# Opendigitalradio/ODR-AudioEnc

Measured on AMD Instinct MI355X. Metric: real-time stereo DAB MP2 streams sustained (frames/s) @128 kbps/48 kHz, higher is better.
Workload: dtype f64; 1 GPU; 4096 streams/GPU x 48 kHz stereo (mode 's') x 128 kbps, psy 1, full encode (BASELINE configs[1]), 32 frames/stream/step; streams_per_gpu=4096, parallelism=streams sharded over 1 GPU(s), no data-path collective

## Files before the change

### odr-audioenc_amd/csrc/mp2_alloc.h

```cpp
#ifndef MP2_WAVE_PARTS
#error "include mp2_wave.h"
#endif
TL_FN int tl_allocate(const TlBlockShared *TL_RESTRICT B, int adb, int nch, int sblimit, int jsbound, PARG(int, a_ln), PARG(int, a_nbal),
                      PARG(int, a_sfs), PARG(int, a_sfs_o), PARG(double, a_smr), PARG(int, ba))
{
    PV(uint64_t, ukey); PV(uint64_t, ukey2); PV(int, nbits); PV(int, cost); PV(int, cost2);
    PV(int, jpair);
    TL_LANES_BEGIN
    const int c = lane & 1, sb = lane >> 1;
    const bool live = c < nch && sb < sblimit;
    const int maxa = (1 << L(a_nbal)) - 1;
    L(ukey) = live ? tl_mnr_key(B->snr_line[L(a_ln)][0] - L(a_smr)) : ~0ull;
    L(ukey2) = (live && 1 < maxa) ? tl_mnr_key(B->snr_line[L(a_ln)][1] - L(a_smr)) : ~0ull;
    L(ba) = 0;
    L(nbits) = (sb < sblimit && c < (sb < jsbound ? nch : 1)) ? L(a_nbal) : 0;
    L(cost) = live ? B->bits12_line[L(a_ln)][1] + 2 + L(a_sfs) + ((nch == 2 && sb >= jsbound) ? 2 + L(a_sfs_o) : 0) : 0;
    L(cost2) = live ? B->bits12_line[L(a_ln)][2] - B->bits12_line[L(a_ln)][1] : 0;
    L(jpair) = (live && nch == 2 && sb >= jsbound) ? 1 : 0;
    TL_LANES_END
    const int bbal = TL_WAVE_SUM_I32(nbits);
    const int ad = adb - (bbal + 16 + 32);
    int spent = 0;
    const bool any_pair = nch == 2 && jsbound < sblimit;
    for (; TL_ENC_LEVEL < 4;) {
        PV(uint64_t, keff); PV(uint64_t, k2eff);
        TL_LANES_BEGIN L(keff) = L(ukey); L(k2eff) = L(ukey2); TL_LANES_END
        if (any_pair) {
            PV(uint64_t, ok1); PV(uint64_t, ok2);
            TL_SWAP1_U64(ok1, ukey); TL_SWAP1_U64(ok2, ukey2);
            TL_LANES_BEGIN
            if (L(jpair)) { if (L(ok1) < L(keff)) L(keff) = L(ok1); if (L(ok2) < L(k2eff)) L(k2eff) = L(ok2); }
            TL_LANES_END
        }
        const uint64_t M = TL_WAVE_MIN_U64(k2eff);
        PV(bool, inb); PV(int, bcost);
        TL_LANES_BEGIN
        L(inb) = L(keff) < M;
        L(bcost) = (L(inb) && !(L(jpair) && (lane & 1))) ? L(cost) : 0;
        TL_LANES_END
        const uint64_t bm = TL_BALLOT(inb);
        if (bm == 0ull) break;
        const int csum = TL_WAVE_SUM_I32(bcost);
        bool last_round = false;
        if (csum > ad - spent) {
            PV(int, pre); PV(int, kh); PV(int, kl); PV(uint64_t, kb);
            TL_LANES_BEGIN L(pre) = 0; L(kh) = (int)(uint32_t)(L(keff) >> 32); L(kl) = (int)(uint32_t)L(keff); L(kb) = L(keff) + 1; TL_LANES_END
            uint64_t pm = bm;
            while (pm) {
                const int j = __builtin_ctzll(pm);
                pm &= pm - 1;
                const int cj = TL_READLANE_I32(bcost, j);
                if (cj == 0) continue;
                const uint64_t kj = ((uint64_t)(uint32_t)TL_READLANE_I32(kh, j) << 32) | (uint32_t)TL_READLANE_I32(kl, j);
                TL_LANES_BEGIN
                if (kj < L(kb)) L(pre) += cj;
                TL_LANES_END
            }
            TL_LANES_BEGIN
            L(inb) = L(inb) && L(pre) <= ad - spent;
            L(bcost) = L(inb) ? L(bcost) : 0;
            TL_LANES_END
            if (TL_BALLOT(inb) == 0ull) break;
            spent += TL_WAVE_SUM_I32(bcost);
            last_round = true;
        } else spent += csum;
        TL_LANES_BEGIN
        if (L(inb)) {
            const int nba = L(ba) + 1;
            L(ba) = nba;
            L(ukey) = L(ukey2);
            L(cost) = L(cost2);
            L(ukey2) = (nba + 1 >= (1 << L(a_nbal)) - 1) ? ~0ull : tl_mnr_key(B->snr_line[L(a_ln)][(nba + 1) & 15] - L(a_smr));
            L(cost2) = B->bits12_line[L(a_ln)][(nba + 2) & 15] - B->bits12_line[L(a_ln)][(nba + 1) & 15];
        }
        TL_LANES_END
        if (last_round) break;
    }
    for (; TL_ENC_LEVEL < 4;) {
        PV(uint64_t, key);
        TL_LANES_BEGIN
        L(key) = L(cost) <= ad - spent ? L(ukey) : ~0ull;
        TL_LANES_END
        const int wl = TL_WAVE_ARGMIN_U64(key);
        if (wl < 0) break;
        const int min_sb = wl >> 1;
        spent += TL_READLANE_I32(cost, wl);
        const bool joint_pair = (min_sb >= jsbound && nch == 2);
        TL_LANES_BEGIN
        if (lane == wl || (joint_pair && (lane ^ 1) == wl)) {
            const int nba = L(ba) + 1;
            L(ba) = nba;
            L(ukey) = L(ukey2);
            L(cost) = L(cost2);
            L(ukey2) = (nba + 1 >= (1 << L(a_nbal)) - 1) ? ~0ull : tl_mnr_key(B->snr_line[L(a_ln)][(nba + 1) & 15] - L(a_smr));
            L(cost2) = B->bits12_line[L(a_ln)][(nba + 2) & 15] - B->bits12_line[L(a_ln)][(nba + 1) & 15];
        }
        TL_LANES_END
    }
    return ad - spent;
}

TL_FN void tl_allocate_pair(const TlBlockShared *TL_RESTRICT B, int adb0, int adb1, int sblimit, PARG(int, a_ln), PARG(int, a_nbal),
                            PARG(int, a_sfs), PARG(double, a_smr), PARG(int, ba))
{
    PV(uint64_t, ukey); PV(uint64_t, ukey2); PV(int, nbits); PV(int, cost); PV(int, cost2); PV(int, room); PV(int, ph); PV(int, bbal);
    TL_LANES_BEGIN
    const bool live = (lane >> 1) < sblimit;
    const int maxa = (1 << L(a_nbal)) - 1;
    L(ukey) = live ? tl_mnr_key(B->snr_line[L(a_ln)][0] - L(a_smr)) : ~0ull;
    L(ukey2) = (live && 1 < maxa) ? tl_mnr_key(B->snr_line[L(a_ln)][1] - L(a_smr)) : ~0ull;
    L(ba) = 0;
    L(nbits) = live ? L(a_nbal) : 0;
    L(cost) = live ? B->bits12_line[L(a_ln)][1] + 2 + L(a_sfs) : 0;
    L(cost2) = live ? B->bits12_line[L(a_ln)][2] - B->bits12_line[L(a_ln)][1] : 0;
    TL_LANES_END
    TL_PAR_SUM_I32(bbal, nbits);
    TL_LANES_BEGIN
    L(room) = ((lane & 1) ? adb1 : adb0) - (L(bbal) + 16 + 32);
    L(ph) = 0;
    TL_LANES_END
    for (; TL_ENC_LEVEL < 4;) {
        PV(uint64_t, k2); PV(uint64_t, M); PV(bool, inb); PV(int, bcost); PV(int, csum); PV(bool, part);
        TL_LANES_BEGIN L(k2) = L(ph) == 0 ? L(ukey2) : ~0ull; TL_LANES_END
        TL_PAR_MIN_U64(M, k2);
        TL_LANES_BEGIN
        L(inb) = L(ph) == 0 && L(ukey) < L(M);
        L(bcost) = L(inb) ? L(cost) | 0x10000 : 0;
        TL_LANES_END
        if (TL_BALLOT(inb) == 0ull) break;
        TL_PAR_SUM_I32(csum, bcost);
        TL_LANES_BEGIN L(part) = L(ph) == 0 && (L(csum) & 0xffff) > L(room); TL_LANES_END
        if (TL_BALLOT(part) != 0ull) {
            PV(int, pre); PV(int, kh); PV(int, kl); PV(bool, pin);
            TL_LANES_BEGIN
            L(pre) = 0; L(kh) = (int)(uint32_t)(L(ukey) >> 32); L(kl) = (int)(uint32_t)L(ukey); L(pin) = L(inb) && L(part);
            TL_LANES_END
            PV(uint64_t, kb);
            for (int u = 0; u < 2; u++) {
                TL_LANES_BEGIN L(kb) = (lane & 1) == u ? L(ukey) + 1 : 0ull; TL_LANES_END
                uint64_t pm = TL_BALLOT(pin) & (0x5555555555555555ull << u);
                while (pm) {
                    const int j = __builtin_ctzll(pm);
                    pm &= pm - 1;
                    const int cj = TL_READLANE_I32(bcost, j) & 0xffff;
                    const uint64_t kj = ((uint64_t)(uint32_t)TL_READLANE_I32(kh, j) << 32) | (uint32_t)TL_READLANE_I32(kl, j);
                    TL_LANES_BEGIN
                    if (kj < L(kb)) L(pre) += cj;
                    TL_LANES_END
                }
            }
            TL_LANES_BEGIN
            if (L(part)) { L(inb) = L(inb) && L(pre) <= L(room); L(bcost) = L(inb) ? L(bcost) : 0; }
            TL_LANES_END
            TL_PAR_SUM_I32(csum, bcost);
        }
        TL_LANES_BEGIN
        if (L(ph) == 0) {
            L(room) -= L(csum) & 0xffff;
            if ((L(csum) >> 16) == 0 || L(part)) L(ph) = 1;
// ... 35 lines not shown
```

### odr-audioenc_amd/csrc/mp2_pack.h

```cpp
#ifndef MP2_WAVE_PARTS
#error "include mp2_wave.h"
#endif
struct TlFrameOut { uint8_t *bytes; uint32_t *words; uint8_t *scfcrc; };
template <int PSY, int NCH = 0>
TL_FN void tl_encode_frame(TlMainLds &w, const TlTables *TL_RESTRICT T, const TlBlockShared *TL_RESTRICT B,
                           const TlConfig *TL_RESTRICT C, const TlPsyOut *TL_RESTRICT PO,
                           const TlPcmView &pv, int xpad_len, const TlFrameOut &fo,
                           const double *TL_RESTRICT enw_s, const TlPackTables *TL_RESTRICT K, int padding, TlTaps *taps, long long *sp)
{
    constexpr int FB = TlMainLds::kFbBatch;
    const int nch = NCH ? NCH : C->nch, sblimit = C->sblimit;
    PA(double, smp, 36);
    PA(int, scf, 3);

    TL_STAMP(sp, 0);
    TL_PRIO2(TL_PS_FB);
    tl_filterbank(w, B, enw_s, nch, smp);

    TL_STAMP(sp, 1);
    TL_PRIO2(1);
#if !defined(TL_EMULATE) && TL_ENC_LEVEL >= 5
    for (int b = 0; b < 36; b++) TL_KEEP(smp[b]);
    scf[0] = scf[1] = scf[2] = 0;
#endif
// ... 81 lines not shown
            w.smr[c][sb] = top - m;
        }
        TL_LANES_END
    }

    TL_STAMP(sp, 3);
    TL_LANES_BEGIN
    const int c = lane & 1, sb = lane >> 1;
    if (TL_ENC_LEVEL < 5 && c < nch && sb < sblimit) {
        int s0 = L(scf)[0], s1 = L(scf)[1], s2 = L(scf)[2];
        int d0 = s0 - s1, d1 = s1 - s2;
        int c0 = d0 <= -3 ? 0 : d0 < 0 ? 1 : d0 == 0 ? 2 : d0 < 3 ? 3 : 4;
        int c1 = d1 <= -3 ? 0 : d1 < 0 ? 1 : d1 == 0 ? 2 : d1 < 3 ? 3 : 4;
        const unsigned p = B->sfpat[c0 * 5 + c1];
        const int m02 = s0 > s2 ? s2 : s0;
        const unsigned q0 = p & 3u, q1 = (p >> 2) & 3u, q2 = (p >> 4) & 3u;
        const int n0 = q0 == 0 ? s0 : q0 == 1 ? s1 : q0 == 2 ? s2 : m02;
        const int n1 = q1 == 0 ? s0 : q1 == 1 ? s1 : q1 == 2 ? s2 : m02;
        const int n2 = q2 == 0 ? s0 : q2 == 1 ? s1 : q2 == 2 ? s2 : m02;
        const int sel = (int)(p >> 6);
        s0 = n0; s1 = n1; s2 = n2;
        L(scf)[0] = s0; L(scf)[1] = s1; L(scf)[2] = s2;
        w.scf[c][0][sb] = (uint8_t)s0; w.scf[c][1][sb] = (uint8_t)s1; w.scf[c][2][sb] = (uint8_t)s2;
        w.scfsi[c][sb] = (uint8_t)sel;
    } else w.scfsi[c][sb] = 0;
    w.balloc[c][sb] = 0;
    TL_LANES_END

    const int lg_frame = C->frame_bytes + padding;
    int adb = lg_frame * 8 - (C->dab_ext * 8 + (xpad_len ? xpad_len : 2) * 8);
    int mode = C->mode0, mode_ext = C->mode_ext0, jsbound = C->jsbound0;
    PV(int, a_sfs); PV(int, a_sfs_o); PV(double, a_smr); PV(double, a_smr_o);
    TL_LANES_BEGIN
    const int c = lane & 1, sb = lane >> 1;
    const bool live = c < nch && sb < sblimit;
    L(a_sfs) = live ? 6 * tl_sfs_count(w.scfsi[c][sb]) : 0;
    L(a_sfs_o) = (live && nch == 2) ? 6 * tl_sfs_count(w.scfsi[1 - c][sb]) : 0;
    L(a_smr) = live ? w.smr[c][sb] : 0.0;
    L(a_smr_o) = (live && nch == 2) ? w.smr[1 - c][sb] : 0.0;
    TL_LANES_END
    if (TL_ENC_LEVEL < 4 && C->mode0 == 1) {
        PV(int, nz_own); PV(int, nz_jnt);
        TL_LANES_BEGIN
        int bo = 0, bj = 0;
        if (lane < 2 * sblimit) {
            const int ln = L(a_ln), maxAlloc = (1 << L(a_nbal)) - 1;
            double sv[15];
#pragma unroll
            for (int q = 0; q < 15; q++) sv[q] = B->snr_line[ln][q];
            int n1 = 0, n2 = 0;
#pragma unroll
            for (int q = 0; q < 15; q++) {
                const bool inr = q < maxAlloc - 1;
                n1 += (inr && !((sv[q] - L(a_smr)) >= 0.0)) ? 1 : 0;
                n2 += (inr && !((sv[q] - L(a_smr_o)) >= 0.0)) ? 1 : 0;
            }
            n2 = n2 > n1 ? n2 : n1;
            bo = n1 > 0 ? B->bits12_line[ln][n1] + 2 + L(a_sfs) : 0;
            bj = n2 > 0 ? B->bits12_line[ln][n2] + 4 + L(a_sfs) + L(a_sfs_o) : 0;
        }
        L(nz_own) = bo; L(nz_jnt) = bj;
        TL_LANES_END
        mode = 0; mode_ext = 0; jsbound = sblimit;
        int tries = 0, try_ext = 4;
        for (;;) {
            PV(int, need);
            TL_LANES_BEGIN
            const int c = lane & 1, sb = lane >> 1;
            int bitsn = 0;
            if (sb < sblimit && c < (sb < jsbound ? nch : 1))
                bitsn = ((nch == 2 && sb >= jsbound) ? L(nz_jnt) : L(nz_own)) + L(a_nbal);
            L(need) = bitsn;
            TL_LANES_END
            int rq = 32 + 16 + TL_WAVE_SUM_I32(need);
            if (tries == 0) {
                if (rq > adb) { mode = 1; } else break;
            } else if (!(rq > adb && try_ext > 0)) { mode_ext = try_ext; break; }
            --try_ext; jsbound = 4 * (try_ext + 1); tries++;
        }
    }
    int adb_left;
    {
        PV(int, ba);
        adb_left = tl_allocate(B, adb, nch, sblimit, jsbound, a_ln, a_nbal, a_sfs, a_sfs_o, a_smr, ba);
        TL_LANES_BEGIN
        const int c = lane & 1, sb = lane >> 1;
        w.balloc[c][sb] = (uint8_t)((c < nch && sb < sblimit) ? L(ba) : 0);
        TL_LANES_END
    }

    TL_STAMP(sp, 4);
    uint32_t *frame = w.u.frame[0];
    TL_LANES_BEGIN
    for (int i = lane; i < ((lg_frame + 3) >> 2) + 2; i += 64) frame[i] = 0;
    TL_LANES_END
    PV(int, f_ba); PV(int, f_sel); PV(int, f_scf); PV(int, f_smp);
    PV(int, o_ba); PV(int, o_sel); PV(int, o_scf); PV(int, o_smp);
    TL_LANES_BEGIN
    const int c = lane & 1, sb = lane >> 1;
    const bool live = c < nch && sb < sblimit;
    const int ba = live ? w.balloc[c][sb] : 0;
    const bool own = sb < sblimit && c < (sb < jsbound ? nch : 1);
    L(f_ba) = own ? L(a_nbal) : 0;
    L(f_sel) = (live && ba) ? 2 : 0;
    L(f_scf) = (live && ba) ? 6 * tl_sfs_count(w.scfsi[c][sb]) : 0;
    L(f_smp) = (own && ba) ? B->bits12_line[L(a_ln)][ba] / 12 : 0;
    TL_LANES_END
    TL_WAVE_EXSCAN_I32(o_ba, f_ba); TL_WAVE_EXSCAN_I32(o_sel, f_sel);
    TL_WAVE_EXSCAN_I32(o_scf, f_scf); TL_WAVE_EXSCAN_I32(o_smp, f_smp);
    const int n_ba = TL_WAVE_SUM_I32(f_ba), n_sel = TL_WAVE_SUM_I32(f_sel);
    const int n_scf = TL_WAVE_SUM_I32(f_scf), n_smp = TL_WAVE_SUM_I32(f_smp);
    const int p_ba = 48, p_sel = p_ba + n_ba, p_scf = p_sel + n_sel, p_smp = p_scf + n_scf;

    if (TL_ENC_LEVEL < 3) {
    TL_LANES_BEGIN
    const int c = lane & 1, sb = lane >> 1;
    if (lane == 0) {
        uint32_t h = (0xfffu << 20) | ((uint32_t)C->version << 19) | (2u << 17) | (0u << 16)
                   | ((uint32_t)C->br_idx << 12) | ((uint32_t)C->fs_idx << 10) | ((uint32_t)padding << 9) | (0u << 8)
                   | ((uint32_t)mode << 6) | ((uint32_t)mode_ext << 4);
        TL_ATOMIC_OR(&frame[0], h);
    }
    const bool live = c < nch && sb < sblimit;
    const int ba = live ? w.balloc[c][sb] : 0;
    if (L(f_ba)) tl_put_bits48(frame, p_ba + L(o_ba), (uint64_t)ba, L(f_ba));
    if (L(f_sel)) {
        const unsigned si = w.scfsi[c][sb];
        tl_put_bits48(frame, p_sel + L(o_sel), si, 2);
        const unsigned s0 = (unsigned)L(scf)[0], s1 = (unsigned)L(scf)[1], s2 = (unsigned)L(scf)[2];
        const unsigned f3 = (s0 << 12) | (s1 << 6) | s2, f2 = (s0 << 6) | s2;
        tl_put_bits48(frame, p_scf + L(o_scf), si == 0 ? f3 : si == 2 ? s0 : f2, L(f_scf));
    }
    TL_LANES_END
    }

    TL_PRIO2(TL_PS_Q);
    if (TL_ENC_LEVEL < 2) {
        const bool any_joint = (nch == 2) && jsbound < sblimit;
        PV(int, q_ba); PV(int, q_nb); PV(int, q_grp); PV(int, q_s2n); PV(int, q_steps);
        PV(double, q_a); PV(double, q_b); PV(double, q_s2nf); PA(double, q_sf, 3); PA(double, q_rsf, 3);
        TL_LANES_BEGIN
        const int c = lane & 1, sb = lane >> 1;
        const bool own = sb < sblimit && c < (sb < jsbound ? nch : 1);
        const int ba = own ? w.balloc[c][sb] : 0;
        const unsigned qi = ba ? B->qinfo_line[L(a_ln)][ba] : 0u;
        const int q = (int)(qi & 31u);
        const bool joint = any_joint && sb >= jsbound;
        L(q_ba) = ba; L(q_nb) = (int)((qi >> 5) & 31u); L(q_grp) = ((qi >> 10) & 1u) ? 3 : 1; L(q_s2n) = K->steps2n[q];
        L(q_steps) = ((qi >> 10) & 1u) ? 1 << L(q_nb) : K->steps[q];
        L(q_a) = K->qa[q]; L(q_b) = K->qb[q]; L(q_s2nf) = K->steps2n_f[q];
        for (int gr = 0; gr < 3; gr++) {
            L(q_sf)[gr] = B->scalefactor[joint ? w.jscale[gr][sb] : L(scf)[gr]];
            L(q_rsf)[gr] = 1.0 / L(q_sf)[gr];
        }
        TL_LANES_END
        uint64_t q_mask = 0;
        int q_n = 64;
        if (TL_Q_REDEAL && !any_joint && !taps) {
            PV(bool, q_live);
            TL_LANES_BEGIN L(q_live) = L(q_ba) != 0; TL_LANES_END
            q_mask = TL_BALLOT(q_live);
            q_n = (int)__builtin_popcountll(q_mask);
        }
        const bool redeal = q_n <= TL_Q_REDEAL_MAX;
        TL_DBG_REDEAL(redeal, q_ba);
        if (redeal) {
            TlQCell *const qc = TL_QRD_CELLS(w);
// ... 521 lines not shown
```

### odr-audioenc_amd/csrc/mp2_probe_stage.h

```cpp
#pragma once
#include "mp2_host.h"
#include "mp2_wave.h"

enum {
    TLS_ADD_DB = 0,
    TLS_MASK,
    TLS_MNR_KEY,
    TLS_SF_INDEX,
    TLS_DIV_BY,
    TLS_LANE_FORMS,
    TLS_SPANS = TLS_LANE_FORMS,
    TLS_MIN_ROWS,
    TLS_BITS,
    TLS_ALLOC,
    TLS_NFORMS
};
#define TLS_LIST 192
#define TLS_ROWS 136
#define TLS_FIELDS 6
#define TLS_FRAME_WORDS (TL_MAX_FRAME_WORDS + 2)
#define TLS_CRC16_POLY 0x8005u
#define TLS_CRC16_TOP 0x8000u
#define TLS_CRC8_POLY 0x1du
#define TLS_CRC8_TOP 0x80u
// ... 205 lines not shown
TL_FN void tl_probe_stage_case(int form, TlStageLds &w, long k, const void *in0, const void *in1, const void *in2, void *out0, void *out1)
{
    const int32_t *ic = (const int32_t *)in2;
    switch (form) {
    case TLS_SPANS: {
        const double *list = (const double *)in0 + TLS_LIST * k, *bnd = (const double *)in1 + 128 * k;
        const int ntone = TL_UNI_I(ic[2 * k]), nnoise = TL_UNI_I(ic[2 * k + 1]), nm = ntone + nnoise;
        TL_LANES_BEGIN
        for (int q = lane; q < TL_MASKER_MAX; q += 64) TL_MK_X(w)[q] = 0.0;
        for (int q = lane; q < TLS_LIST; q += 64) TL_MK_BARK(w)[q] = list[q];
        TL_LANES_END
        TL_LANES_BEGIN
        for (int t = lane; t < TL_MASKER_MAX; t += 64) {
            if (t < nm) tl_masker_consts(TL_MK4(w), TL_MK_X(w), TL_MK_BARK(w), t, t < ntone);
            else TL_MK4(w)[t].bark = TL_MK_BARK(w)[t];
        }
        TL_LANES_END
        const bool sorted = tl_maskers_sorted(TL_MK_BARK(w), ntone, nnoise);
        const bool srt = ntone < 128 && nnoise < 64 && sorted;
        TL_LANES_BEGIN
        const double blo = bnd[2 * lane], bhi = bnd[2 * lane + 1];
        int32_t *o = (int32_t *)out0 + 512 * k + 8 * lane;
        int a0, a1, b0, b1;
        tl_mask_spans(TL_MK4(w), nm, ntone, blo, bhi, a0, a1, b0, b1);
        o[0] = a0; o[1] = a1; o[2] = b0; o[3] = b1;
        a0 = a1 = b0 = b1 = -2;
        if (srt) tl_mask_spans_sorted<64, 32>(TL_MK_BARK(w), ntone, nnoise, blo, bhi, a0, a1, b0, b1);
        o[4] = a0; o[5] = a1; o[6] = b0; o[7] = b1;
        if (lane == 0) { ((int32_t *)out1)[2 * k] = sorted ? 1 : 0; ((int32_t *)out1)[2 * k + 1] = srt ? 1 : 0; }
        TL_LANES_END
    } break;
    case TLS_MIN_ROWS: {
        const double *col = (const double *)in0 + TLS_ROWS * k, *m0 = (const double *)in1 + 64 * k;
        TL_LANES_BEGIN
        for (int q = lane; q < TLS_ROWS; q += 64) TL_LTG(w)[q] = col[q];
        TL_LANES_END
        TL_LANES_BEGIN
        const int32_t *r = ic + 192 * k + 3 * lane;
        ((double *)out0)[64 * k + lane] = tl_min_rows(TL_LTG(w), r[0], r[1], m0[lane], r[2] != 0);
        TL_LANES_END
    } break;
    case TLS_BITS: {
        const uint64_t *val = (const uint64_t *)in0 + 64 * TLS_FIELDS * k;
        const int32_t *len = (const int32_t *)in1 + 64 * TLS_FIELDS * k;
        const int start = TL_UNI_I(ic[2 * k]), wide = TL_UNI_I(ic[2 * k + 1]);
        uint32_t *frame = w.frame;
        PV(int, tot); PV(int, off);
        TL_LANES_BEGIN
        for (int q = lane; q < TLS_FRAME_WORDS; q += 64) frame[q] = 0;
        int t = 0;
        for (int f = 0; f < TLS_FIELDS; f++) t += len[TLS_FIELDS * lane + f];
        L(tot) = t;
        TL_LANES_END
        TL_WAVE_EXSCAN_I32(off, tot);
        TL_LANES_BEGIN
        int pos = start + L(off);
        unsigned c16 = 0xffffu, c8 = 0;
        for (int f = 0; f < TLS_FIELDS; f++) {
            const uint64_t v = val[TLS_FIELDS * lane + f];
            const int nb = len[TLS_FIELDS * lane + f];
            if (wide) { if (nb) tl_put_bits48(frame, pos, v, nb); }
            else tl_put_bits(frame, pos, (uint32_t)v, nb);
            const int hi = nb > 32 ? nb - 32 : 0;
            c16 = tl_crc_upd(c16, (unsigned)(v >> 32), hi, TLS_CRC16_POLY, TLS_CRC16_TOP); c16 = tl_crc_upd(c16, (unsigned)v, nb - hi, TLS_CRC16_POLY, TLS_CRC16_TOP);
            c8 = tl_crc_upd(c8, (unsigned)(v >> 32), hi, TLS_CRC8_POLY, TLS_CRC8_TOP); c8 = tl_crc_upd(c8, (unsigned)v, nb - hi, TLS_CRC8_POLY, TLS_CRC8_TOP);
            pos += nb;
        }
        ((uint32_t *)out1)[128 * k + 2 * lane] = c16 & 0xffffu; ((uint32_t *)out1)[128 * k + 2 * lane + 1] = c8 & 0xffu;
        TL_LANES_END
        TL_LANES_BEGIN
        uint32_t *o = (uint32_t *)out0 + 3 * TLS_FRAME_WORDS * k;
        for (int q = lane; q < TLS_FRAME_WORDS; q += 64) {
            const uint32_t word = frame[q];
            uint32_t u = 0;
            for (int bit = 0; bit < 32; bit++) u = (u << 1) | tl_get_bit(frame, 32 * q + bit);
            o[q] = word; o[TLS_FRAME_WORDS + q] = u; o[2 * TLS_FRAME_WORDS + q] = tl_bswap(word);
        }
        TL_LANES_END
    } break;
    default: break;
    }
}

TL_FN void tl_probe_alloc_case(const TlBlockShared *TL_RESTRICT B, const TlsAllocTab *TL_RESTRICT A, long k, const void *in0, const void *in1, const void *in2, void *out0, void *out1)
{
    const int32_t *ic = (const int32_t *)in2;
    const double *smr = (const double *)in0 + 64 * k;
    const int32_t *sel = (const int32_t *)in1 + 64 * k, *p = ic + 8 * k;
    const int tab = TL_UNI_I(p[0]), nch = TL_UNI_I(p[1]), jsbound = TL_UNI_I(p[2]), call = TL_UNI_I(p[3]), adb0 = TL_UNI_I(p[4]), adb1 = TL_UNI_I(p[5]);
    const int sblimit = TL_UNI_I(A->sblimit[tab]);
    PV(int, a_ln); PV(int, a_nbal); PV(int, a_sfs); PV(int, a_sfs_o); PV(double, a_smr); PV(int, ba);
    int left = 0;
    if (call == 0) {
        TL_LANES_BEGIN
        const int c = lane & 1, sb = lane >> 1;
        const bool live = c < nch && sb < sblimit;
        L(a_ln) = live ? A->line[tab][sb] : 0;
        L(a_nbal) = live ? A->nbal[tab][sb] : 0;
        L(a_sfs) = live ? 6 * tl_sfs_count((unsigned)sel[lane]) : 0;
        L(a_sfs_o) = (live && nch == 2) ? 6 * tl_sfs_count((unsigned)sel[lane ^ 1]) : 0;
        L(a_smr) = live ? smr[lane] : 0.0;
        TL_LANES_END
        left = tl_allocate(B, adb0, nch, sblimit, jsbound, a_ln, a_nbal, a_sfs, a_sfs_o, a_smr, ba);
    } else {
        TL_LANES_BEGIN
        const int sb = lane >> 1;
        const bool live = sb < sblimit;
        L(a_ln) = live ? A->line[tab][sb] : 0;
        L(a_nbal) = live ? A->nbal[tab][sb] : 0;
        L(a_sfs) = live ? 6 * tl_sfs_count((unsigned)sel[lane]) : 0;
        L(a_smr) = live ? smr[lane] : 0.0;
        TL_LANES_END
        tl_allocate_pair(B, adb0, adb1, sblimit, a_ln, a_nbal, a_sfs, a_smr, ba);
    }
    TL_LANES_BEGIN
    ((int32_t *)out0)[64 * k + lane] = L(ba);
    if (lane == 0) ((int32_t *)out1)[k] = left;
    TL_LANES_END
}
```

### odr-audioenc_amd/csrc/mp2_wave.h

```cpp
#pragma once
#include "mp2_types.h"
#include "tl_libm.h"
#include <math.h>
#include <stddef.h>

#ifdef TL_EMULATE
#define TL_FN static inline
#define TL_LANES_BEGIN for (int lane = 0; lane < 64; ++lane) {
#define TL_LANES_END }
#define TL_SYNC() ((void)0)
#define PV(T, name) T name[64]
#define PA(T, name, n) T name[64][n]
#define L(name) name[lane]
#define PARG(T, name) T (&name)[64]
#define PARGA(T, name, n) T (&name)[64][n]
#define TL_OTHER(name, idx, src) name[src] idx
#define TL_ATOMIC_OR(p, v) (*(p) |= (v))
TL_FN uint64_t tlh_ballot(const bool (&p)[64]) { uint64_t m = 0; for (int i = 0; i < 64; i++) if (p[i]) m |= 1ull << i; return m; }
TL_FN uint64_t tlh_min_u64(const uint64_t (&v)[64]) { uint64_t m = v[0]; for (int i = 1; i < 64; i++) if (v[i] < m) m = v[i]; return m; }
TL_FN int tlh_sum_i32(const int (&v)[64]) { int s = 0; for (int i = 0; i < 64; i++) s += v[i]; return s; }
TL_FN uint32_t tlh_xor_u32(const uint32_t (&v)[64]) { uint32_t s = 0; for (int i = 0; i < 64; i++) s ^= v[i]; return s; }
TL_FN void tlh_exscan_i32(int (&d)[64], const int (&v)[64]) { int s = 0; for (int i = 0; i < 64; i++) { d[i] = s; s += v[i]; } }
TL_FN int tlh_argmin_u64(const uint64_t (&v)[64])
{
    const uint64_t m = tlh_min_u64(v);
    if (m == ~0ull) return -1;
    for (int i = 0; i < 64; i += 2) if (v[i] == m) return i;
    for (int i = 1; i < 64; i += 2) if (v[i] == m) return i;
    return -1;
}
TL_FN void tlh_row16_max_f64(double (&d)[64], const double (&v)[64])
{ for (int r = 0; r < 4; r++) { double m = v[16 * r]; for (int i = 1; i < 16; i++) if (!(v[16 * r + i] < m)) m = v[16 * r + i]; for (int i = 0; i < 16; i++) d[16 * r + i] = m; } }
#define TL_ROW16_MAX_F64(dst, src) tlh_row16_max_f64(dst, src)
TL_FN void tlh_incl_xscan_u32(uint32_t (&d)[64], const uint32_t (&v)[64]) { uint32_t x = 0; for (int i = 0; i < 64; i++) { x ^= v[i]; d[i] = x; } }
#define TL_WAVE_INCL_XSCAN_U32(dst, src) tlh_incl_xscan_u32(dst, src)
TL_FN void tlh_par_min_u64(uint64_t (&d)[64], const uint64_t (&v)[64])
{ for (int p = 0; p < 2; p++) { uint64_t m = v[p]; for (int i = p; i < 64; i += 2) if (v[i] < m) m = v[i]; for (int i = p; i < 64; i += 2) d[i] = m; } }
TL_FN void tlh_par_sum_i32(int (&d)[64], const int (&v)[64])
{ for (int p = 0; p < 2; p++) { int m = 0; for (int i = p; i < 64; i += 2) m += v[i]; for (int i = p; i < 64; i += 2) d[i] = m; } }
#define TL_PAR_MIN_U64(dst, src) tlh_par_min_u64(dst, src)
#define TL_PAR_SUM_I32(dst, src) tlh_par_sum_i32(dst, src)
#define TL_BALLOT(name) tlh_ballot(name)
#define TL_SWAP1_U64(dst, src) do { for (int l_ = 0; l_ < 64; l_++) dst[l_] = src[l_ ^ 1]; } while (0)
#define TL_SWAP1_F64(dst, di, src, si) do { for (int l_ = 0; l_ < 64; l_++) dst[l_] di = src[l_ ^ 1] si; } while (0)
#define TL_SPLAT(dst, di, val) do { for (int l_ = 0; l_ < 64; l_++) dst[l_] di = (val); } while (0)
#define TL_ROT32_F64(dst, src) do { for (int l_ = 0; l_ < 64; l_++) dst[l_] = src[(l_ + 32) & 63]; } while (0)
#define TL_MIRROR_SB_F64(dst, src, n) do { for (int l_ = 0; l_ < 64; l_++) for (int k_ = 0; k_ < (n); k_++) dst[l_][k_] = src[2 * (31 - (l_ >> 1)) + (l_ & 1)][k_]; } while (0)
#define TL_WAVE_ARGMIN_U64(name) tlh_argmin_u64(name)
#define TL_WAVE_MIN_U64(name) tlh_min_u64(name)
#define TL_WAVE_SUM_I32(name) tlh_sum_i32(name)
#define TL_WAVE_XOR_U32(name) tlh_xor_u32(name)
#define TL_WAVE_EXSCAN_I32(dst, src) tlh_exscan_i32(dst, src)
#define TL_UNI_I(x) (x)
#define TL_READLANE_I32(name, l) name[l]
#define TL_RESTRICT
#define TL_SELECT(c, a, b) ((c) ? (a) : (b))
#define TL_LAUNDER(p) ((void)0)
#define TL_KARG const TlLaunch *
#define TL_KEEP(x) ((void)0)
#define TL_PIN(x) ((void)0)
#define TL_TIE(p, v) ((void)0)
#define TL_LD2(p, a, b) do { const double *p_ = (p); (a) = p_[0]; (b) = p_[1]; } while (0)
#define TL_ST2(p, a, b) do { double *p_ = (p); p_[0] = (a); p_[1] = (b); } while (0)
#define TL_RANK_BELOW(mask) __builtin_popcountll((mask) & ((1ull << lane) - 1ull))
TL_FN int tl_sign_bit(double x) { return (int)(tl_d2u(x) >> 63); }
#define TL_SCHED_FENCE() ((void)0)
#define TL_SCT(t, row, j) ((t)[(row) + (j)])
#else
#define TL_FN __device__ __forceinline__
#define TL_LANES_BEGIN { int lane_ = (int)(threadIdx.x & 63u); asm volatile("" : "+v"(lane_)); __builtin_assume(lane_ >= 0 && lane_ < 64); const int lane = lane_;
#define TL_LANES_END } TL_SYNC();
#define TL_SYNC() do { __builtin_amdgcn_fence(__ATOMIC_RELEASE, "wavefront"); __builtin_amdgcn_wave_barrier(); \
                       __builtin_amdgcn_fence(__ATOMIC_ACQUIRE, "wavefront"); } while (0)
#define PV(T, name) T name
#define PA(T, name, n) T name[n]
#define L(name) name
#define PARG(T, name) T &name
#define PARGA(T, name, n) T (&name)[n]
#define TL_OTHER(name, idx, src) tld_shfl_f64(name idx, src)
#define TL_ATOMIC_OR(p, v) atomicOr((p), (v))
TL_FN double tld_shfl_f64(double v, int src) { return __shfl(v, src, 64); }
TL_FN double tld_swap1_f64(double v) {
    const uint64_t u = tl_d2u(v);
    const uint32_t lo = (uint32_t)__builtin_amdgcn_update_dpp(0, (int)(uint32_t)u, 0xB1, 0xf, 0xf, true);
    const uint32_t hi = (uint32_t)__builtin_amdgcn_update_dpp(0, (int)(uint32_t)(u >> 32), 0xB1, 0xf, 0xf, true);
    return tl_u2d(((uint64_t)hi << 32) | lo);
}
struct TldMin { template <class T> static TL_FN T f(T a, T b) { return a < b ? a : b; } };
struct TldAdd { template <class T> static TL_FN T f(T a, T b) { return a + b; } };
struct TldXor { template <class T> static TL_FN T f(T a, T b) { return a ^ b; } };
template <class OP, class T> TL_FN T tld_ladder(T v, const T id)
{
    v = OP::f((T)__builtin_amdgcn_update_dpp((int)id, (int)v, 0x111, 0xf, 0xf, false), v);
    v = OP::f((T)__builtin_amdgcn_update_dpp((int)id, (int)v, 0x112, 0xf, 0xf, false), v);
    v = OP::f((T)__builtin_amdgcn_update_dpp((int)id, (int)v, 0x114, 0xf, 0xf, false), v);
    v = OP::f((T)__builtin_amdgcn_update_dpp((int)id, (int)v, 0x118, 0xf, 0xf, false), v);
    v = OP::f((T)__builtin_amdgcn_update_dpp((int)id, (int)v, 0x142, 0xa, 0xf, false), v);
    v = OP::f((T)__builtin_amdgcn_update_dpp((int)id, (int)v, 0x143, 0xc, 0xf, false), v);
    return v;
}
TL_FN uint32_t tld_min_u32(uint32_t v) { return (uint32_t)__builtin_amdgcn_readlane((int)tld_ladder<TldMin>(v, 0xffffffffu), 63); }
TL_FN uint64_t tld_min_u64(uint64_t v) {
    const uint32_t hi = (uint32_t)(v >> 32), lo = (uint32_t)v;
    const uint32_t mhi = tld_min_u32(hi);
    const uint32_t mlo = tld_min_u32(hi == mhi ? lo : 0xffffffffu);
    return ((uint64_t)mhi << 32) | mlo;
}
TL_FN int tld_incl_scan_i32(int v) { return tld_ladder<TldAdd>(v, 0); }
TL_FN uint32_t tld_incl_xscan_u32(uint32_t x) { return tld_ladder<TldXor>(x, 0u); }
#define TL_WAVE_INCL_XSCAN_U32(dst, src) dst = tld_incl_xscan_u32(src)
TL_FN uint32_t tld_xor_u32(uint32_t x) { return (uint32_t)__builtin_amdgcn_readlane((int)tld_incl_xscan_u32(x), 63); }
TL_FN int tld_sum_i32(int v) { return __builtin_amdgcn_readlane(tld_incl_scan_i32(v), 63); }
TL_FN int tld_exscan_i32(int v) { return tld_incl_scan_i32(v) - v; }
TL_FN int tld_argmin_u64(uint64_t v)
{
    const uint32_t hi = (uint32_t)(v >> 32), lo = (uint32_t)v;
    const uint32_t mhi = tld_min_u32(hi);
    uint64_t m = (uint64_t)__ballot(hi == mhi);
    if (__builtin_popcountll(m) > 1) {
        const uint32_t mlo = tld_min_u32(hi == mhi ? lo : 0xffffffffu);
        if ((mhi & mlo) == 0xffffffffu) return -1;
        m = (uint64_t)__ballot(hi == mhi && lo == mlo);
    } else if (mhi == 0xffffffffu && (uint32_t)__builtin_amdgcn_readlane((int)lo, __builtin_ctzll(m)) == 0xffffffffu) return -1;
    const uint64_t even = m & 0x5555555555555555ull;
    return __builtin_ctzll(even ? even : m);
}
template <int SH> TL_FN double tld_row_shr_f64(double v)
{
    const uint64_t u = tl_d2u(v);
    const uint32_t lo = (uint32_t)__builtin_amdgcn_update_dpp((int)(uint32_t)u, (int)(uint32_t)u, 0x110 | SH, 0xf, 0xf, false);
    const uint32_t hi = (uint32_t)__builtin_amdgcn_update_dpp((int)(uint32_t)(u >> 32), (int)(uint32_t)(u >> 32), 0x110 | SH, 0xf, 0xf, false);
    return tl_u2d(((uint64_t)hi << 32) | lo);
}
TL_FN double tld_row16_max_f64(double v)
{
    double o;
    o = tld_row_shr_f64<1>(v); v = v < o ? o : v;
    o = tld_row_shr_f64<2>(v); v = v < o ? o : v;
    o = tld_row_shr_f64<4>(v); v = v < o ? o : v;
    o = tld_row_shr_f64<8>(v); v = v < o ? o : v;
    return v;
}
#define TL_ROW16_MAX_F64(dst, src) dst = tld_row16_max_f64(src)
TL_FN uint32_t tld_par_min_u32(uint32_t v)
{
    uint32_t t;
    t = (uint32_t)__builtin_amdgcn_update_dpp((int)v, (int)v, 0x122, 0xf, 0xf, false); v = t < v ? t : v;
    t = (uint32_t)__builtin_amdgcn_update_dpp((int)v, (int)v, 0x124, 0xf, 0xf, false); v = t < v ? t : v;
    t = (uint32_t)__builtin_amdgcn_update_dpp((int)v, (int)v, 0x128, 0xf, 0xf, false); v = t < v ? t : v;
    const auto r = __builtin_amdgcn_permlane16_swap(v, v, false, false); v = r[0] < r[1] ? r[0] : r[1];
    const auto q = __builtin_amdgcn_permlane32_swap(v, v, false, false); v = q[0] < q[1] ? q[0] : q[1];
    return v;
}
TL_FN uint64_t tld_par_min_u64(uint64_t v)
{
    const uint32_t hi = (uint32_t)(v >> 32), lo = (uint32_t)v;
    const uint32_t mhi = tld_par_min_u32(hi);
    const uint32_t mlo = tld_par_min_u32(hi == mhi ? lo : 0xffffffffu);
    return ((uint64_t)mhi << 32) | mlo;
}
TL_FN int tld_par_sum_i32(int v)
{
    v += __builtin_amdgcn_update_dpp(v, v, 0x122, 0xf, 0xf, false);
// ... 227 lines not shown
```

### odr-audioenc_amd/csrc/toolame_probe.hip

```cpp
#include <hip/hip_runtime.h>
#include <math.h>
#include <vector>
#include "mp2_host.h"
#include "mp2_probe.h"
#include "tlb_debug.h"
#include "tlb_mem.h"

__global__ void __launch_bounds__(256) tl_probe_libm_kernel(int form, int table, long n, const double *a, const double *b, double *r0, double *r1)
{
    __shared__ TlProbeTables t;
    tl_probe_fill_tables(t, (int)threadIdx.x, 256);
    __syncthreads();
    const long i0 = (long)blockIdx.x * 256 + (long)(threadIdx.x & ~63u);
    if (i0 >= n) return;
    if (table) tl_probe_libm_unit(form, t.lt, t.sct, i0, n, a, b, r0, r1);
    else tl_probe_libm_unit(form, tlm_log_tab, t.sct, i0, n, a, b, r0, r1);
}

__global__ void __launch_bounds__(256) tl_probe_wave_kernel(int prim, int nwaves, const uint64_t *in, const uint64_t *in2, uint64_t *out)
{
    __shared__ __attribute__((aligned(16))) double pair[4][128];
    const int wave = (int)(threadIdx.x >> 6), w = (int)blockIdx.x * 4 + wave;
    if (w >= nwaves) return;
    tl_probe_wave_unit(prim, in + (size_t)w * 64 * tlp_in_words(prim), in2 + (size_t)w * 64, out + (size_t)w * 64 * tlp_out_words(prim), pair[wave]);
}

__global__ void __launch_bounds__(256) tl_probe_stage_kernel(int form, long n, const double *dblog, const double *sftab, const TlBlockShared *shared,
                                                             const TlsAllocTab *atab, const void *in0, const void *in1, const void *in2, void *out0, void *out1)
{
    static_assert(sizeof(TlBlockShared) % 8 == 0, "copied as doubles");
    __shared__ TlBlockShared blk;
    __shared__ __attribute__((aligned(16))) double dbt[1002];
    __shared__ __attribute__((aligned(16))) double sfl[64];
    __shared__ TlStageLds lds[4];
    for (int i = (int)threadIdx.x; i < 1002; i += 256) dbt[i] = dblog[i];
    if (threadIdx.x < 64) sfl[threadIdx.x] = sftab[threadIdx.x];
    if (form == TLS_ALLOC) for (int i = (int)threadIdx.x; i < (int)(sizeof(TlBlockShared) / 8); i += 256) ((double *)&blk)[i] = ((const double *)shared)[i];
    __syncthreads();
    const int wave = (int)(threadIdx.x >> 6);
    if (form < TLS_LANE_FORMS) {
        const long i0 = (long)blockIdx.x * 256 + 64 * wave;
        if (i0 >= n) return;
        tl_probe_stage_lanes(form, lds[wave], dbt, sfl, i0, n, in0, in1, in2, out0, out1);
    } else {
        const long k = (long)blockIdx.x * 4 + wave;
        if (k >= n) return;
        if (form == TLS_ALLOC) tl_probe_alloc_case(&blk, atab, k, in0, in1, in2, out0, out1);
        else tl_probe_stage_case(form, lds[wave], k, in0, in1, in2, out0, out1);
    }
}

#ifdef TLB_FAULT_INJECT
#define TLP_MAX_N (1l << 26)
#define TLP_HIP(x) do { if ((x) != hipSuccess) return TLB_ERR_HIP; } while (0)

extern "C" int tlb_debug_probe_libm(int form, int table, long n, const double *a, const double *b, double *r0, double *r1)
{
    if (form < 0 || form >= TLP_NFORMS || n <= 0 || n > TLP_MAX_N || !a || !r0) return TLB_ERR_ARG;
    if (table != 0 && !(table == 1 && tlp_has_table(form))) return TLB_ERR_ARG;
    const bool in2 = tlp_two_in(form), out2 = tlp_two_out(form);
    if ((in2 && !b) || (out2 && !r1)) return TLB_ERR_ARG;
    for (long i = 0; i < n; i++) if (!tlp_in_domain(form, a[i], in2 ? b[i] : 0.0)) return TLB_ERR_ARG;
    const size_t bytes = (size_t)n * sizeof(double);
    TlbMem m;
    double *da = m.scratch<double>((size_t)n), *db = m.dev<double>((size_t)n), *d0 = m.dev<double>((size_t)n), *d1 = m.dev<double>((size_t)n);
    m.upload(da, a, bytes);
    if (in2) m.upload(db, b, bytes);
    if (!m.settle()) return TLB_ERR_HIP;
    tl_probe_libm_kernel<<<dim3((unsigned)((n + 255) / 256)), dim3(256), 0, 0>>>(form, table, n, da, db, d0, d1);
    TLP_HIP(hipGetLastError());
    TLP_HIP(hipDeviceSynchronize());
    TLP_HIP(hipMemcpy(r0, d0, bytes, hipMemcpyDeviceToHost));
    if (out2) TLP_HIP(hipMemcpy(r1, d1, bytes, hipMemcpyDeviceToHost));
    return TLB_OK;
}

extern "C" int tlb_debug_probe_wave(int prim, int nwaves, const void *in, const void *in2, void *out)
{
    if (prim < 0 || prim >= TLP_NPRIMS || nwaves <= 0 || nwaves > (1 << 20) || !in || !out) return TLB_ERR_ARG;
    const bool two = tlp_wave_two_in(prim);
    if (two && !in2) return TLB_ERR_ARG;
    const size_t iw = (size_t)64 * tlp_in_words(prim), ow = (size_t)64 * tlp_out_words(prim), nw = (size_t)nwaves;
    const uint64_t *hin = (const uint64_t *)in, *hin2 = (const uint64_t *)in2;
    for (size_t w = 0; w < nw; w++) if (!tlp_wave_case_ok(prim, hin + w * iw, two ? hin2 + w * 64 : nullptr)) return TLB_ERR_ARG;
    TlbMem m;
    uint64_t *di = m.scratch<uint64_t>(nw * iw), *di2 = m.dev<uint64_t>(nw * 64), *dout = m.dev<uint64_t>(nw * ow);
    m.upload(di, in, nw * iw * 8);
    if (two) m.upload(di2, in2, nw * 64 * 8);
    if (!m.settle()) return TLB_ERR_HIP;
    tl_probe_wave_kernel<<<dim3((unsigned)((nwaves + 3) / 4)), dim3(256), 0, 0>>>(prim, nwaves, di, di2, dout);
    TLP_HIP(hipGetLastError());
    TLP_HIP(hipDeviceSynchronize());
    TLP_HIP(hipMemcpy(out, dout, nw * ow * 8, hipMemcpyDeviceToHost));
    return TLB_OK;
}

extern "C" int tlb_debug_probe_stage(int form, long n, const void *in0, const void *in1, const void *in2, void *out0, void *out1)
{
    if (form < 0 || form >= TLS_NFORMS || n <= 0 || n > tls_max_n(form)) return TLB_ERR_ARG;
    size_t by[5];
    tls_bytes(form, n, by);
    const void *hin[3] = {in0, in1, in2};
    void *hout[2] = {out0, out1};
    for (int k = 0; k < 3; k++) if (by[k] && !hin[k]) return TLB_ERR_ARG;
    for (int k = 0; k < 2; k++) if (by[3 + k] && !hout[k]) return TLB_ERR_ARG;
    if (!tls_in_domain(form, n, in0, in1, in2)) return TLB_ERR_ARG;
    static TlTables T;
    static bool built = false;
    if (!built) { tl_build_tables(&T); built = true; }
    std::vector<double> recip;
    if (form == TLS_DIV_BY) {
        recip.resize((size_t)n);
        for (long i = 0; i < n; i++) recip[(size_t)i] = 1.0 / ((const double *)in1)[i];
        hin[2] = recip.data(); by[2] = 8 * (size_t)n;
    }
    TlbMem m;
    double *ddb = m.scratch<double>(1002), *dsf = m.scratch<double>(64);
    m.upload(ddb, T.dblog, 1002 * sizeof(double));
    m.upload(dsf, T.shared.scalefactor, 64 * sizeof(double));
    TlBlockShared *dsh = m.scratch<TlBlockShared>(1);
    TlsAllocTab *dat = m.scratch<TlsAllocTab>(1);
    m.upload(dsh, &T.shared, sizeof(TlBlockShared));
    if (form == TLS_ALLOC) m.upload(dat, tls_alloc_tab(), sizeof(TlsAllocTab));
    char *din[3], *dout[2];
    for (int k = 0; k < 3; k++) { din[k] = m.dev<char>(by[k]); if (by[k]) m.upload(din[k], hin[k], by[k]); }
    for (int k = 0; k < 2; k++) dout[k] = m.dev<char>(by[3 + k]);
    if (!m.settle()) return TLB_ERR_HIP;
    const long per = form < TLS_LANE_FORMS ? 256 : 4;
    tl_probe_stage_kernel<<<dim3((unsigned)((n + per - 1) / per)), dim3(256), 0, 0>>>(form, n, ddb, dsf, dsh, dat, din[0], din[1], din[2], dout[0], dout[1]);
    TLP_HIP(hipGetLastError());
// ... 6 lines not shown
```

Measured before the change: 37.63 million frames/s.

## Narrow partial-admission allocation round with LDS histogram bucketing before serial prefix scan

When the last greedy bit-allocation round would overflow the budget, the candidate set is first narrowed by up to two passes of a 64-bucket cost histogram over the key range (atomic adds into LDS scratch plus a wave exclusive scan). This finds the cutoff bucket, so only the lanes inside it go through the serial per-lane readlane prefix loop. The aim is to cut the O(popcount) serial loop in the partial round. In exchange it adds LDS atomics, scans and ballots per pass, and reuses the frame buffer as scratch before that buffer is cleared. Emulator-only debug counters and mutant switches are included too.

```diff
diff --git a/odr-audioenc_amd/csrc/mp2_alloc.h b/odr-audioenc_amd/csrc/mp2_alloc.h
--- a/odr-audioenc_amd/csrc/mp2_alloc.h
+++ b/odr-audioenc_amd/csrc/mp2_alloc.h
@@ -1,8 +1,27 @@
 #ifndef MP2_WAVE_PARTS
 #error "include mp2_wave.h"
 #endif
+#ifndef TL_CUT_PASSES
+#define TL_CUT_PASSES 2
+#endif
+#ifndef TL_CUT_SERIAL
+#define TL_CUT_SERIAL 6
+#endif
+enum { TLA_PARTIAL, TLA_FIRST, TLA_EVENTS, TLA_SERIAL, TLA_PASS1, TLA_PASS2, TLA_DEGENERATE, TLA_SMALL, TLA_CUT0, TLA_CUTLAST, TLA_ONEBUCKET, TLA_BELOW, TLA_JOINTCUT, TLA_ADMITTED, TLA_N };
+#ifdef TL_EMULATE
+static long tl_dbg_alloc[TLA_N];
+#define TL_DBG_ALLOC(k, n) (tl_dbg_alloc[k] += (n))
+extern "C" __attribute__((weak, visibility("default"))) void emu_alloc_stats(long *out, int reset)
+{ for (int i = 0; i < TLA_N; i++) { if (out) out[i] = tl_dbg_alloc[i]; if (reset) tl_dbg_alloc[i] = 0; } }
+#else
+#define TL_DBG_ALLOC(k, n) ((void)0)
+#endif
+#if !defined(TL_EMULATE) || !defined(TL_ALLOC_MUTANT)
+#undef TL_ALLOC_MUTANT
+#define TL_ALLOC_MUTANT 0
+#endif
 TL_FN int tl_allocate(const TlBlockShared *TL_RESTRICT B, int adb, int nch, int sblimit, int jsbound, PARG(int, a_ln), PARG(int, a_nbal),
-                      PARG(int, a_sfs), PARG(int, a_sfs_o), PARG(double, a_smr), PARG(int, ba))
+                      PARG(int, a_sfs), PARG(int, a_sfs_o), PARG(double, a_smr), PARG(int, ba), uint32_t *TL_RESTRICT hist)
 {
     PV(uint64_t, ukey); PV(uint64_t, ukey2); PV(int, nbits); PV(int, cost); PV(int, cost2);
     PV(int, jpair);
@@ -22,6 +41,7 @@
     const int ad = adb - (bbal + 16 + 32);
     int spent = 0;
     const bool any_pair = nch == 2 && jsbound < sblimit;
+    uint64_t Mprev = 0;
     for (; TL_ENC_LEVEL < 4;) {
         PV(uint64_t, keff); PV(uint64_t, k2eff);
         TL_LANES_BEGIN L(keff) = L(ukey); L(k2eff) = L(ukey2); TL_LANES_END
@@ -43,9 +63,62 @@
         const int csum = TL_WAVE_SUM_I32(bcost);
         bool last_round = false;
         if (csum > ad - spent) {
-            PV(int, pre); PV(int, kh); PV(int, kl); PV(uint64_t, kb);
-            TL_LANES_BEGIN L(pre) = 0; L(kh) = (int)(uint32_t)(L(keff) >> 32); L(kl) = (int)(uint32_t)L(keff); L(kb) = L(keff) + 1; TL_LANES_END
-            uint64_t pm = bm;
+            PV(int, pre); PV(int, kh); PV(int, kl); PV(uint64_t, kb); PV(bool, cand);
+            const int room = ad - spent;
+            int base = 0;
+            uint64_t pm = bm, lo = Mprev, hi = M - 1;
+            TL_LANES_BEGIN L(cand) = L(inb); TL_LANES_END
+            TL_DBG_ALLOC(TLA_PARTIAL, 1); TL_DBG_ALLOC(TLA_FIRST, spent == 0 ? 1 : 0);
+#ifdef TL_EMULATE
+            for (int l = 0; l < 64; l++) if (inb[l] && bcost[l]) TL_DBG_ALLOC(TLA_EVENTS, 1);
+#endif
+            TL_DBG_ALLOC(TLA_DEGENERATE, hi <= lo ? 1 : 0); TL_DBG_ALLOC(TLA_SMALL, __builtin_popcountll(pm) <= TL_CUT_SERIAL ? 1 : 0);
+#pragma nounroll
+            for (int pass = 0; pass < TL_CUT_PASSES; pass++) {
+                if (hi <= lo || __builtin_popcountll(pm) <= TL_CUT_SERIAL) break;
+                int sh = 58 - __builtin_clzll(hi - lo);
+                sh = sh < 0 ? 0 : sh;
+                if (TL_ALLOC_MUTANT == 4 && sh > 0) sh--;
+                PV(int, bk); PV(int, hw); PV(int, ex); PV(bool, over);
+                TL_LANES_BEGIN
+                L(bk) = (int)((uint32_t)((L(keff) - lo) >> sh) & 63u);
+                hist[lane] = 0;
+                TL_LANES_END
+                TL_LANES_BEGIN
+                if (TL_ALLOC_MUTANT == 3) { if (L(cand)) TL_ATOMIC_ADD(&hist[L(bk)], (uint32_t)L(cost)); }
+                else if (L(cand) && L(bcost) != 0) TL_ATOMIC_ADD(&hist[L(bk)], (uint32_t)L(bcost));
+                TL_LANES_END
+                TL_LANES_BEGIN L(hw) = (int)hist[lane]; TL_LANES_END
+                TL_WAVE_EXSCAN_I32(ex, hw);
+                TL_LANES_BEGIN L(over) = base + L(ex) + L(hw) > room; TL_LANES_END
+                const uint64_t ov = TL_BALLOT(over);
+                if (ov == 0ull) break;
+                const int bs = __builtin_ctzll(ov);
+#ifdef TL_EMULATE
+                {
+                    int top = -1, nb = 0;
+                    for (int l = 0; l < 64; l++) { if (hist[l]) { top = l; nb++; } if (cand[l] && (keff[l] < lo || keff[l] > hi)) TL_DBG_ALLOC(TLA_BELOW, 1); }
+                    TL_DBG_ALLOC(pass ? TLA_PASS2 : TLA_PASS1, 1);
+                    if (pass == 0) { TL_DBG_ALLOC(TLA_CUT0, bs == 0 ? 1 : 0); TL_DBG_ALLOC(TLA_CUTLAST, bs == top ? 1 : 0); TL_DBG_ALLOC(TLA_ONEBUCKET, nb == 1 ? 1 : 0); }
+                }
+#endif
+                base += TL_READLANE_I32(ex, bs);
+                TL_LANES_BEGIN
+                if (L(cand) && !(TL_ALLOC_MUTANT == 1 ? L(bk) < bs : L(bk) <= bs)) L(inb) = false;
+                L(cand) = L(cand) && L(bk) == bs;
+                TL_LANES_END
+                pm = TL_BALLOT(cand);
+                lo += (uint64_t)bs << sh;
+                const uint64_t top = lo + ((1ull << sh) - 1ull);
+                hi = top < hi ? top : hi;
+            }
+#ifdef TL_EMULATE
+            for (int l = 0, jp = 0; l < 64; l++) { if (cand[l] && bcost[l]) TL_DBG_ALLOC(TLA_SERIAL, 1); if (cand[l] && jpair[l] && !jp) { jp = 1; TL_DBG_ALLOC(TLA_JOINTCUT, 1); } }
+#endif
+            TL_LANES_BEGIN
+            L(pre) = TL_ALLOC_MUTANT == 2 ? 0 : base;
+            L(kh) = (int)(uint32_t)(L(keff) >> 32); L(kl) = (int)(uint32_t)L(keff); L(kb) = L(keff) + 1;
+            TL_LANES_END
             while (pm) {
                 const int j = __builtin_ctzll(pm);
                 pm &= pm - 1;
@@ -57,9 +130,12 @@
                 TL_LANES_END
             }
             TL_LANES_BEGIN
-            L(inb) = L(inb) && L(pre) <= ad - spent;
+            L(inb) = L(inb) && (!L(cand) || L(pre) <= room);
             L(bcost) = L(inb) ? L(bcost) : 0;
             TL_LANES_END
+#ifdef TL_EMULATE
+            for (int l = 0; l < 64; l++) if (inb[l] && bcost[l]) TL_DBG_ALLOC(TLA_ADMITTED, 1);
+#endif
             if (TL_BALLOT(inb) == 0ull) break;
             spent += TL_WAVE_SUM_I32(bcost);
             last_round = true;
@@ -75,6 +151,7 @@
         }
         TL_LANES_END
         if (last_round) break;
+        Mprev = M;
     }
     for (; TL_ENC_LEVEL < 4;) {
         PV(uint64_t, key);
diff --git a/odr-audioenc_amd/csrc/mp2_pack.h b/odr-audioenc_amd/csrc/mp2_pack.h
--- a/odr-audioenc_amd/csrc/mp2_pack.h
+++ b/odr-audioenc_amd/csrc/mp2_pack.h
@@ -187,7 +187,7 @@
     int adb_left;
     {
         PV(int, ba);
-        adb_left = tl_allocate(B, adb, nch, sblimit, jsbound, a_ln, a_nbal, a_sfs, a_sfs_o, a_smr, ba);
+        adb_left = tl_allocate(B, adb, nch, sblimit, jsbound, a_ln, a_nbal, a_sfs, a_sfs_o, a_smr, ba, w.u.frame[0]);
         TL_LANES_BEGIN
         const int c = lane & 1, sb = lane >> 1;
         w.balloc[c][sb] = (uint8_t)((c < nch && sb < sblimit) ? L(ba) : 0);
diff --git a/odr-audioenc_amd/csrc/mp2_probe_stage.h b/odr-audioenc_amd/csrc/mp2_probe_stage.h
--- a/odr-audioenc_amd/csrc/mp2_probe_stage.h
+++ b/odr-audioenc_amd/csrc/mp2_probe_stage.h
@@ -311,8 +311,13 @@
     }
 }
 
-TL_FN void tl_probe_alloc_case(const TlBlockShared *TL_RESTRICT B, const TlsAllocTab *TL_RESTRICT A, long k, const void *in0, const void *in1, const void *in2, void *out0, void *out1)
-{
+TL_FN void tl_probe_alloc_case(const TlBlockShared *TL_RESTRICT B, const TlsAllocTab *TL_RESTRICT A, long k, const void *in0, const void *in1, const void *in2, void *out0, void *out1,
+                               uint32_t *hist = nullptr)
+{
+#ifdef TL_EMULATE
+    uint32_t hist_own[64];
+    if (!hist) hist = hist_own;
+#endif
     const int32_t *ic = (const int32_t *)in2;
     const double *smr = (const double *)in0 + 64 * k;
     const int32_t *sel = (const int32_t *)in1 + 64 * k, *p = ic + 8 * k;
@@ -330,7 +335,7 @@
         L(a_sfs_o) = (live && nch == 2) ? 6 * tl_sfs_count((unsigned)sel[lane ^ 1]) : 0;
         L(a_smr) = live ? smr[lane] : 0.0;
         TL_LANES_END
-        left = tl_allocate(B, adb0, nch, sblimit, jsbound, a_ln, a_nbal, a_sfs, a_sfs_o, a_smr, ba);
+        left = tl_allocate(B, adb0, nch, sblimit, jsbound, a_ln, a_nbal, a_sfs, a_sfs_o, a_smr, ba, hist);
     } else {
         TL_LANES_BEGIN
         const int sb = lane >> 1;
diff --git a/odr-audioenc_amd/csrc/mp2_wave.h b/odr-audioenc_amd/csrc/mp2_wave.h
--- a/odr-audioenc_amd/csrc/mp2_wave.h
+++ b/odr-audioenc_amd/csrc/mp2_wave.h
@@ -16,6 +16,7 @@
 #define PARGA(T, name, n) T (&name)[64][n]
 #define TL_OTHER(name, idx, src) name[src] idx
 #define TL_ATOMIC_OR(p, v) (*(p) |= (v))
+#define TL_ATOMIC_ADD(p, v) (*(p) += (v))
 TL_FN uint64_t tlh_ballot(const bool (&p)[64]) { uint64_t m = 0; for (int i = 0; i < 64; i++) if (p[i]) m |= 1ull << i; return m; }
 TL_FN uint64_t tlh_min_u64(const uint64_t (&v)[64]) { uint64_t m = v[0]; for (int i = 1; i < 64; i++) if (v[i] < m) m = v[i]; return m; }
 TL_FN int tlh_sum_i32(const int (&v)[64]) { int s = 0; for (int i = 0; i < 64; i++) s += v[i]; return s; }
@@ -79,6 +80,7 @@
 #define PARGA(T, name, n) T (&name)[n]
 #define TL_OTHER(name, idx, src) tld_shfl_f64(name idx, src)
 #define TL_ATOMIC_OR(p, v) atomicOr((p), (v))
+#define TL_ATOMIC_ADD(p, v) atomicAdd((p), (v))
 TL_FN double tld_shfl_f64(double v, int src) { return __shfl(v, src, 64); }
 TL_FN double tld_swap1_f64(double v) {
     const uint64_t u = tl_d2u(v);
diff --git a/odr-audioenc_amd/csrc/toolame_probe.hip b/odr-audioenc_amd/csrc/toolame_probe.hip
--- a/odr-audioenc_amd/csrc/toolame_probe.hip
+++ b/odr-audioenc_amd/csrc/toolame_probe.hip
@@ -45,7 +45,7 @@
     } else {
         const long k = (long)blockIdx.x * 4 + wave;
         if (k >= n) return;
-        if (form == TLS_ALLOC) tl_probe_alloc_case(&blk, atab, k, in0, in1, in2, out0, out1);
+        if (form == TLS_ALLOC) tl_probe_alloc_case(&blk, atab, k, in0, in1, in2, out0, out1, lds[wave].frame);
         else tl_probe_stage_case(form, lds[wave], k, in0, in1, in2, out0, out1);
     }
 }
```

After: 38.07 million frames/s, median of 6. 1.01x the previous value.
